# ZihanLiao/pytorch-kaldi-resnet

Hardware: AMD Instinct MI355X
Metric: utterances/sec (300-frame x 80 fbank, bs256/GPU), ResNet-34 + AAM-softmax training step (higher is better)
Workload: dtype f32 (operands as 2 fp16 terms of value x 2^k, 3 cross products, f32 accumulate); 1 GPU; BASELINE configs[1]: ResNet-34 + AAM-softmax (m 0.2, s 30), 1211 speakers, 300-frame x 80 fbank, per-GPU batch 256, fwd+CE+bwd+SGD(0.9, wd 5e-4); global_batch=256, frames=300, feat_dim=80, parallelism=dp1, launch=hipGraph replay (1 graph), mfma=f16x3

## Files before the change

include/spkhip.h:

```cpp
#ifndef SPKHIP_H
#define SPKHIP_H
#include <stddef.h>
#ifdef __cplusplus
extern "C" {
#endif

int spk_version(void);
const char* spk_last_error(void);
int spk_build_flags(void);

#define SPK_IN_AFFINE_RELU 1
#define SPK_EPI_AFFINE 2
#define SPK_EPI_ADD 4
#define SPK_EPI_RELU 8
#define SPK_EPI_STATS 16
#define SPK_IN_BNBWD 64
#define SPK_EPI_BNBWD 32

#define SPK_CONV_WS 128
#define SPK_CONV_PIPE 1024

#define SPK_CONV_M16 (1 << 17)

#define SPK_WGRAD_GROUPS 2048
// ... 77 lines not shown
size_t spk_bn_finalize_workspace(int nblk, int C);
int spk_bn_finalize(const float* partial, int nblk, int C, double count, const float* gamma, const float* beta,
                    float* running_mean, float* running_var, long long* num_batches_tracked, float* mean, float* invstd,
                    float* scale, float* shift, float momentum, float eps, double* ws,
                    const unsigned* amax_in, unsigned* est_out ,
                    void* stream);
int spk_bn_eval_coeffs(const float* gamma, const float* beta, const float* running_mean, const float* running_var,
                       float* scale, float* shift, int C, float eps, void* stream);
int spk_bn_apply(const float* raw, const float* scale, const float* shift, const float* res, const float* res_scale,
                 const float* res_shift, float* out, unsigned* mask_out, long long N, int C, int relu,
                 unsigned* amax_out , void* stream);
int spk_bn_bwd_reduce(const float* dy, const float* raw, const float* act, const float* mean, const float* invstd,
                      const float* scale, const float* shift, float* partial, long long N, int C, int mask_mode,
                      unsigned* chan_amax , void* stream);
int spk_bn_bwd_finalize(const float* partial, int nblk, int C, double count, const float* gamma, const float* invstd,
                        float* dgamma, float* dbeta, float* coef , int accumulate, double* ws,
                        const unsigned* amax_in, const unsigned* raw_amax, const float* mean, unsigned* est_out ,
                        const unsigned* chan_amax ,
                        void* stream);
int spk_bn_bwd_apply(const float* dy, const float* raw, const float* act, const float* mean, const float* invstd,
                     const float* scale, const float* shift, const float* coef, float* draw, float* dz_out, long long N,
                     int C, int mask_mode, unsigned* amax_out ,
                     const unsigned* pair_scale , void* stream);
int spk_absmax(const float* x, unsigned* slot, long long n, void* stream);
int spk_bnbwd_estimate(const float* coef, const float* mean, const float* invstd, int C, const unsigned* amax_in,
                       const unsigned* raw_amax, unsigned* est, void* stream);
int spk_f16_window_count(const float* x, const float* scale, const float* shift, long long n, int C, const unsigned* slot,
                         int pairs, unsigned long long* counts , void* stream);
int spk_affine_estimate(const float* scale, const float* shift, int C, const unsigned* amax_in, unsigned* est, void* stream);

int spk_se_chunks(long long HW);
int spk_se_squeeze(const float* x, float* partial, double* sums , int B, int H, int W, int C, const int* wlen,
                   void* stream);
int spk_se_excite(const double* sums, const float* scale, const float* shift, const float* W1, const float* W2, float* q,
                  float* u, float* g, int B, int C, int Cr, int H, int W, const int* wlen, void* stream);
int spk_se_apply(const float* raw, const float* scale, const float* shift, const float* gate, const float* res,
                 const float* res_scale, const float* res_shift, float* out, unsigned* mask_out, int B, int H, int W, int C,
                 int relu, unsigned* amax_out, const int* wlen, void* stream);
int spk_se_bwd_reduce(const float* dout, const float* raw, const float* act, float* partial, double* S , int B,
                      long long HW, int C, int mask_mode, unsigned* chan_amax, void* stream);
int spk_se_bwd_gate(const double* S, const double* sums, const float* q, const float* u, const float* g, const float* W1,
                    const float* W2, const float* mean, const float* invstd, const float* scale, const float* shift,
                    const float* gamma, float* da, float* du, float* dq, float* dW1, float* dW2, float* dgamma, float* dbeta,
                    float* coef, int accumulate, int B, int C, int Cr, long long HW, const unsigned* amax_in,
                    const unsigned* raw_amax, const unsigned* chan_amax, unsigned* est_out, void* stream);
int spk_se_bwd_apply(const float* dout, const float* raw, const float* act, const float* gate, const float* dqs ,
// ... 118 lines not shown
```

pytorch-kaldi-resnet_amd/csrc/bn.hip:

```cpp
#include "spk_common.h"

enum { MASK_NONE = 0, MASK_ACT = 1, MASK_RAW = 2, MASK_BITS = 3 };

__global__ __launch_bounds__(256) void bn_stats_partial_kernel(const float* __restrict__ x, float* __restrict__ partial,
                                                               long long N, int C, int rows_per_block) {
    __shared__ float red[256][8];
    const int tid = threadIdx.x;
    const int qpr = C >> 2;
    const int quad = tid % qpr, prow = tid / qpr, rstep = 256 / qpr;
    const long long r0 = (long long)blockIdx.x * rows_per_block;
    long long r1 = r0 + rows_per_block;
    if (r1 > N) r1 = N;
    f32x4 s = {0.f, 0.f, 0.f, 0.f}, ss = {0.f, 0.f, 0.f, 0.f};
    for (long long r = r0 + prow; r < r1; r += rstep) {
        const f32x4 v = *(const f32x4*)(x + r * C + quad * 4);
        s += v;
        ss += v * v;
    }
#pragma unroll
    for (int k = 0; k < 4; ++k) {
        red[tid][k] = s[k];
        red[tid][4 + k] = ss[k];
    }
    __syncthreads();
// ... 286 lines not shown
                bits |= __shfl_xor(bits, 4, 64);
                if ((threadIdx.x & 7) == 0) mask_out[i >> 3] = bits;
            }
        }
    }
    if (amax_out) spk_wave_amax_commit(mx, amax_out);
}

extern "C" int spk_bn_apply(const float* raw, const float* scale, const float* shift, const float* res,
                            const float* res_scale, const float* res_shift, float* out, unsigned* mask_out, long long N, int C,
                            int relu, unsigned* amax_out, void* stream) {
    SPK_REQUIRE(raw && scale && shift && out, "spk_bn_apply: null pointer");
    SPK_REQUIRE(N > 0 && bn_c_ok(C), "spk_bn_apply: N=%lld C=%d", N, C);
    SPK_REQUIRE((res_scale == nullptr) == (res_shift == nullptr), "spk_bn_apply: residual affine must come in pairs");
    SPK_REQUIRE(!res_scale || res, "spk_bn_apply: residual affine without residual");
    SPK_REQUIRE(!mask_out || C % 32 == 0, "spk_bn_apply: the sign mask needs C %% 32 == 0 (C=%d)", C);
    const long long nquads = N * C / 4;
    hipLaunchKernelGGL(bn_apply_kernel, dim3(stream_grid(nquads, BN_APPLY_U, BN_APPLY_CAP)), dim3(256), 0, (hipStream_t)stream, raw, scale, shift, res,
                       res_scale, res_shift, out, mask_out, nquads, C, relu, amax_out);
    SPK_LAUNCH_CHECK("spk_bn_apply");
    return 0;
}

__device__ inline f32x4 bn_mask(f32x4 dy, int mode, const float* act, const float* raw_p, f32x4 rawv, f32x4 sc, f32x4 sh,
                                long long off, int C = 0) {
    if (mode == MASK_BITS) {
        const int lg = 31 - __builtin_clz((unsigned)C);
        const long long pix = off >> lg;
        const int c = (int)(off & (C - 1));
        const unsigned bits = ((const unsigned*)act)[pix * (C >> 5) + (c >> 5)] >> (c & 31);
#pragma unroll
        for (int k = 0; k < 4; ++k) dy[k] = ((bits >> k) & 1u) ? dy[k] : 0.f;
    } else if (mode == MASK_ACT) {
        const f32x4 a = *(const f32x4*)(act + off);
#pragma unroll
        for (int k = 0; k < 4; ++k) dy[k] = a[k] > 0.f ? dy[k] : 0.f;
    } else if (mode == MASK_RAW) {
        const f32x4 z = rawv * sc + sh;
#pragma unroll
        for (int k = 0; k < 4; ++k) dy[k] = z[k] > 0.f ? dy[k] : 0.f;
    }
    (void)raw_p;
    return dy;
}

__global__ __launch_bounds__(256) void bn_bwd_reduce_kernel(const float* __restrict__ dy, const float* __restrict__ raw,
                                                            const float* __restrict__ act, const float* __restrict__ mean,
                                                            const float* __restrict__ invstd, const float* __restrict__ scale,
                                                            const float* __restrict__ shift, float* __restrict__ partial,
                                                            long long N, int C, int rows_per_block, int mode,
                                                            unsigned* __restrict__ chan_amax) {
    __shared__ float red[256][8];
    const int tid = threadIdx.x;
    const int qpr = C >> 2;
    const int quad = tid % qpr, prow = tid / qpr, rstep = 256 / qpr;
    const long long r0 = (long long)blockIdx.x * rows_per_block;
    long long r1 = r0 + rows_per_block;
    if (r1 > N) r1 = N;
    const f32x4 mu = *(const f32x4*)(mean + quad * 4), is = *(const f32x4*)(invstd + quad * 4);
    const f32x4 sc = *(const f32x4*)(scale + quad * 4), sh = *(const f32x4*)(shift + quad * 4);
    f32x4 s = {0.f, 0.f, 0.f, 0.f}, ss = {0.f, 0.f, 0.f, 0.f}, mx = {0.f, 0.f, 0.f, 0.f};
    for (long long r = r0 + prow; r < r1; r += rstep) {
        const long long off = r * C + quad * 4;
        const f32x4 rv = ld_stream(raw + off);
        f32x4 d = ld_stream(dy + off);
        d = bn_mask(d, mode, act, raw, rv, sc, sh, off, C);
        const f32x4 xh = (rv - mu) * is;
        s += d;
        ss += d * xh;
#pragma unroll
        for (int k = 0; k < 4; ++k) mx[k] = fmaxf(mx[k], spk_finite_abs(d[k]));
    }
#pragma unroll
    for (int k = 0; k < 4; ++k) {
        red[tid][k] = s[k];
        red[tid][4 + k] = ss[k];
    }
    __syncthreads();
    if (tid < qpr) {
        float a[8];
#pragma unroll
        for (int k = 0; k < 8; ++k) a[k] = 0.f;
        for (int p = 0; p < rstep; ++p)
#pragma unroll
            for (int k = 0; k < 8; ++k) a[k] += red[p * qpr + tid][k];
        float* dst = partial + ((size_t)blockIdx.x * C + tid * 4) * 2;
#pragma unroll
        for (int k = 0; k < 4; ++k) {
            dst[k * 2 + 0] = a[k];
            dst[k * 2 + 1] = a[4 + k];
        }
    }
    if (chan_amax) {
        __syncthreads();
#pragma unroll
        for (int k = 0; k < 4; ++k) red[tid][k] = mx[k];
        __syncthreads();
        if (tid < qpr) {
#pragma unroll
            for (int k = 0; k < 4; ++k) {
                float m = 0.f;
                for (int p = 0; p < rstep; ++p) m = fmaxf(m, red[p * qpr + tid][k]);
                const unsigned bits = __float_as_uint(m);
                unsigned* slot = chan_amax + tid * 4 + k;
                if (bits > __hip_atomic_load(slot, __ATOMIC_RELAXED, __HIP_MEMORY_SCOPE_AGENT)) atomicMax(slot, bits);
            }
        }
    }
}

extern "C" int spk_bn_bwd_reduce(const float* dy, const float* raw, const float* act, const float* mean, const float* invstd,
                                 const float* scale, const float* shift, float* partial, long long N, int C, int mask_mode,
                                 unsigned* chan_amax, void* stream) {
    SPK_REQUIRE(dy && raw && mean && invstd && scale && shift && partial, "spk_bn_bwd_reduce: null pointer");
    SPK_REQUIRE(N > 0 && bn_c_ok(C), "spk_bn_bwd_reduce: N=%lld C=%d", N, C);
    SPK_REQUIRE(mask_mode >= 0 && mask_mode <= 3, "spk_bn_bwd_reduce: mask_mode=%d", mask_mode);
    SPK_REQUIRE((mask_mode != MASK_ACT && mask_mode != MASK_BITS) || act, "spk_bn_bwd_reduce: MASK_ACT / MASK_BITS need the activated tensor / its sign bits");
    const int nb = spk_bn_stats_blocks(N, C);
    const int rpb = (int)((N + nb - 1) / nb);
    hipLaunchKernelGGL(bn_bwd_reduce_kernel, dim3(nb), dim3(256), 0, (hipStream_t)stream, dy, raw, act, mean, invstd, scale,
                       shift, partial, N, C, rpb, mask_mode, chan_amax);
    SPK_LAUNCH_CHECK("spk_bn_bwd_reduce");
    return 0;
}

__device__ inline float bnbwd_bound(float k1, float m1, float m2, float mean, float invstd, float A, float R) {
    const float xh = (R + fabsf(mean)) * fabsf(invstd);
    return fabsf(k1) * (A + fabsf(m1) + xh * fabsf(m2)) * (1.f + 1.52587890625e-05f);
}

template <typename T>
__global__ __launch_bounds__(256) void bn_bwd_finalize_kernel(const T* __restrict__ partial, int nblk, int C, double count,
                                                              const float* __restrict__ gamma, const float* __restrict__ invstd,
                                                              float* __restrict__ dgamma, float* __restrict__ dbeta,
                                                              float* __restrict__ coef, int accumulate,
                                                              const unsigned* __restrict__ amax_in, const unsigned* __restrict__ raw_amax,
                                                              const float* __restrict__ mean, unsigned* __restrict__ est_out,
                                                              const unsigned* __restrict__ chan_amax) {
    __shared__ double red[8][32][2];
    const int tid = threadIdx.x, c = tid & 31, row = tid >> 5;
    const int ch = blockIdx.x * 32 + c;
    double s = 0.0, ss = 0.0;
    if (ch < C) bn_sum_rows<T>(partial, nblk, C, ch, row, s, ss);
    red[row][c][0] = s;
    red[row][c][1] = ss;
// ... 117 lines not shown
            } else
                st_stream(draw + off, o);
            mx = fmaxf(fmaxf(mx, fmaxf(fabsf(o[0]), fabsf(o[1]))), fmaxf(fabsf(o[2]), fabsf(o[3])));
        }
    }
    if (amax_out) spk_wave_amax_commit(mx, amax_out);
}

extern "C" int spk_bn_bwd_apply(const float* dy, const float* raw, const float* act, const float* mean, const float* invstd,
                                const float* scale, const float* shift, const float* coef, float* draw, float* dz_out,
                                long long N, int C, int mask_mode, unsigned* amax_out, const unsigned* pair_scale, void* stream) {
    SPK_REQUIRE(dy && raw && mean && invstd && scale && shift && coef && draw, "spk_bn_bwd_apply: null pointer");
    SPK_REQUIRE(N > 0 && bn_c_ok(C), "spk_bn_bwd_apply: N=%lld C=%d", N, C);
    SPK_REQUIRE(mask_mode >= 0 && mask_mode <= 3, "spk_bn_bwd_apply: mask_mode=%d", mask_mode);
    SPK_REQUIRE((mask_mode != MASK_ACT && mask_mode != MASK_BITS) || act, "spk_bn_bwd_apply: MASK_ACT / MASK_BITS need the activated tensor / its sign bits");
    const long long nquads = N * C / 4;
    SPK_REQUIRE(nquads < 2147483647LL / 8, "spk_bn_bwd_apply: %lld values exceed the 32-bit group index of the kernel", N * C);
    hipLaunchKernelGGL(bn_bwd_apply_kernel, dim3(stream_grid(nquads, BN_BWD_APPLY_U, BN_BWD_APPLY_CAP)), dim3(256), 0, (hipStream_t)stream, dy, raw, act, mean,
                       invstd, scale, shift, coef, draw, dz_out, (unsigned)nquads, C, mask_mode, amax_out, pair_scale);
    SPK_LAUNCH_CHECK("spk_bn_bwd_apply");
    return 0;
}

__global__ __launch_bounds__(256) void absmax_kernel(const float* __restrict__ x, long long n, unsigned* __restrict__ slot) {
    float mx = 0.f;
    const long long nq = n >> 2;
    for (long long i = (long long)blockIdx.x * 256 + threadIdx.x; i < nq; i += (long long)gridDim.x * 256) {
        const f32x4 v = *(const f32x4*)(x + i * 4);
        mx = fmaxf(fmaxf(mx, fmaxf(spk_finite_abs(v[0]), spk_finite_abs(v[1]))), fmaxf(spk_finite_abs(v[2]), spk_finite_abs(v[3])));
    }
    if (blockIdx.x == 0 && threadIdx.x < (n & 3)) mx = fmaxf(mx, spk_finite_abs(x[nq * 4 + threadIdx.x]));
    spk_wave_amax_commit(mx, slot);
}

extern "C" int spk_absmax(const float* x, unsigned* slot, long long n, void* stream) {
    SPK_REQUIRE(x && slot && n > 0, "spk_absmax: bad arguments");
    SPK_REQUIRE((((size_t)x) & 15) == 0, "spk_absmax: x must be 16-byte aligned");
    hipLaunchKernelGGL(absmax_kernel, dim3(stream_grid(n / 4 + 1)), dim3(256), 0, (hipStream_t)stream, x, n, slot);
    SPK_LAUNCH_CHECK("spk_absmax");
    return 0;
}

__global__ __launch_bounds__(256) void bnbwd_estimate_kernel(const float* __restrict__ coef, const float* __restrict__ mean,
                                                             const float* __restrict__ invstd, int C,
                                                             const unsigned* __restrict__ amax_in, const unsigned* __restrict__ raw_amax,
                                                             unsigned* __restrict__ est) {
// ... 117 lines not shown
```

pytorch-kaldi-resnet_amd/engine.py:

```python
import torch

from . import ops
from .hip import MASK_ACT, MASK_BITS, MASK_NONE, MASK_RAW


class _Conv:
    def __init__(self, holder):
        self.h = holder
        self.cin, self.cout, self.k, self.stride = holder.cin, holder.cout, holder.k, holder.stride
        self.wpk = None
        self.wpk_t = None

    def repack(self, need_t):
        w = self.h.weight.data
        if self.cin == 1:
            return
        self.wpk = ops.pack_conv_weight(w, False, self.wpk)
        if need_t:
            self.wpk_t = ops.pack_conv_weight(w, True, self.wpk_t)

    def pack_jobs(self, need_t):
        w = self.h.weight.data
        if self.cin == 1:
            return []
# ... 74 lines not shown
                self.blocks.append(_Block(bp))
        self.head_bn = _BN(model.bn1) if hasattr(model, "bn1") else None
        self.pool_mode = 1 if model.pooling == "mean+std" else 0
        self.dirty = True
        self._packed_for_bwd = False
        self._pack_tables = {}
        self._amax_pool = None
        self._amax_fwd = None
        self._amax_eval = None
        self._fwd_gen = 0
        self.wgrad_stream = None
        self.use_side_stream = True
        self.fuse_bn_reduce = True
        self.fuse_bn_apply = True
        import os
        self.use_sign_masks = os.environ.get("SPK_SIGN_MASKS", "1") == "1"
        self.fuse_apply_min_c = int(os.environ.get("SPK_FUSE_APPLY_MINC", "0"))
        self._fuse_apply_max_c = int(os.environ["SPK_FUSE_APPLY_MAXC"]) if "SPK_FUSE_APPLY_MAXC" in os.environ else None
        self.fuse_apply_1x1 = os.environ.get("SPK_FUSE_APPLY_1X1", "0") == "1"
        self.pair_draw = os.environ.get("SPK_PAIR_DRAW", "1") == "1"
        stem_fused = os.environ.get("SPK_STEM_FUSED", "1")
        self.stem_fused_fwd = stem_fused in ("1", "fwd")
        self.stem_fused_bwd = stem_fused in ("1", "bwd")
        self.chan_amax = os.environ.get("SPK_CHAN_AMAX", "1") == "1"
        self.window_counts = None
        self.bound_log = None

    @property
    def fuse_apply_max_c(self):
        if self._fuse_apply_max_c is not None:
            return self._fuse_apply_max_c
        return 32 if (self.pair_draw and ops.split_for(3, True) == 3) else 1000000

    @fuse_apply_max_c.setter
    def fuse_apply_max_c(self, v):
        self._fuse_apply_max_c = v

    def _all_convs(self):
        for b in self.blocks:
            for c in b.convs:
                yield c
            if b.ds is not None:
                yield b.ds[0]

    def _repack(self, need_t):
        if not self.dirty and (self._packed_for_bwd or not need_t):
# ... 323 lines not shown
                if on_stage_done and (bi == 0 or stage_of[bi - 1] != stage_of[bi]):
                    self._join_wgrad()
                    on_stage_done("layer%d" % stage_of[bi])
            bn = self.stem_bn
            if self.stem_fused_bwd:
                raw0 = saved["raw0"]
                if part is None:
                    part = ops.bn_bwd_partial(d, raw0, None, bn.t4, MASK_RAW)
                coef = ops.bn_bwd_coef(part, raw0.numel() // raw0.shape[-1], bn.h.weight.data, bn.t4, bn.h.weight.grad,
                                       bn.h.bias.grad, accumulate=acc)
                ops.stem_bwd_wgrad(saved["x"], d, raw0, bn.t4, coef, self.stem_conv.h.weight.grad, accumulate=acc)
            else:
                draw0 = ops.bn_backward(d, saved["raw0"], None, bn.t4, bn.h.weight.data, bn.h.weight.grad, bn.h.bias.grad,
                                        MASK_RAW, draw_out=d, accumulate=acc, partial=part)
                ops.stem_wgrad(saved["x"], draw0, self.stem_conv.h.weight.grad, accumulate=acc)
            self._join_wgrad()
            if on_stage_done:
                on_stage_done("stem")

    def _block_bwd(self, b, rec, dout, acc, dout_partial=None, prev=None, dout_amax=None, amx=None, chan=False):
        x, raws, out = rec["x"], rec["raws"], rec["out"]
        n = len(b.convs)
        g, g_part, g_amax, dz = dout, dout_partial, dout_amax, None
        take = (lambda: amx.take()) if amx is not None else (lambda: None)
        for i in range(n - 1, -1, -1):
            c, bn, raw = b.convs[i], b.bns[i], raws[i]
            last = i == n - 1
            inp = x if i == 0 else raws[i - 1]
            in_aff = None if i == 0 else (b.bns[i - 1].t4[2], b.bns[i - 1].t4[3])
            hw = (inp.shape[1], inp.shape[2])
            act = out if last else None
            f16 = amx is not None and ops.split_for(c.k, True) == 3
            add_dz, bnb = False, None
            if i > 0:
                if c.stride == 1 and self.fuse_bn_reduce:
                    bnb = (raws[i - 1], None, b.bns[i - 1].t4)
            elif b.ds is None:
                add_dz = True
                if c.stride == 1 and self.fuse_bn_reduce and prev is not None:
                    bnb = (prev[0], x, prev[1])
                    if rec.get("xmask") is not None:
                        bnb = bnb + (rec["xmask"],)
            res_amax, draw_amax = take(), take()
            pairs = f16 and self.pair_draw
            raw_amax = rec["raw_amax"][i] if f16 else None
            se_last = last and b.se is not None
# ... 28 lines not shown
                    self.bound_log.append((c.cout, c.k, est, draw_amax))
            else:
                lazy_dz = False
                est = take() if pairs else None
                pair = (g_amax, raw_amax, est) if pairs else None
                if se_last:
                    bits = rec.get("mask")
                    lazy_dz = b.ds is None and bits is not None and n > 1
                    ca = amx.take_n(c.cout) if (chan and pairs) else None
                    mode, actm = (MASK_BITS, bits) if bits is not None else (MASK_ACT, out)
                    sums, q, u, gate = rec["se"]
                    S = ops.se_bwd_reduce(g, raw, actm, mode, chan_amax=ca)
                    w1, w2 = b.se.w1, b.se.w2
                    coef, dq, _, _ = ops.se_bwd_gate(S, sums, q, u, gate, w1.data, w2.data, bn.t4, bn.h.weight.data, w1.grad,
                                                     w2.grad, bn.h.weight.grad, bn.h.bias.grad, raw.shape[1] * raw.shape[2],
                                                     accumulate=acc, pair=pair, chan_amax=ca)
                    draw = ops.se_bwd_apply(g, raw, actm, mode, gate, dq[1], bn.t4, coef, e_out=None if lazy_dz else g,
                                            amax_out=draw_amax, pair_scale=est)
                    dz = None if lazy_dz else g
                elif last:
                    bits = rec.get("mask")
                    lazy_dz = b.ds is None and bits is not None and n > 1
                    ca = amx.take_n(c.cout) if (chan and pairs and g_part is None) else None
                    draw = ops.bn_backward(g, raw, bits if bits is not None else out, bn.t4, bn.h.weight.data, bn.h.weight.grad,
                                           bn.h.bias.grad, MASK_BITS if bits is not None else MASK_ACT,
                                           dz_out=None if lazy_dz else g, accumulate=acc, partial=g_part, amax_out=draw_amax,
                                           pair=pair, chan_amax=ca)
                    dz = None if lazy_dz else g
                else:
                    draw = ops.bn_backward(g, raw, None, bn.t4, bn.h.weight.data, bn.h.weight.grad, bn.h.bias.grad, MASK_RAW,
                                           draw_out=g, accumulate=acc, partial=g_part, amax_out=draw_amax, pair=pair)
                draw_slot = est if pairs else draw_amax
                self._count(draw, draw_slot, pairs=pairs)
                if self.bound_log is not None and est is not None:
                    self.bound_log.append((c.cout, c.k, est, draw_amax))
                if add_dz and dz is None and rec.get("mask") is not None:
                    res = ops.conv_dgrad(draw, c.wpk_t, c.cin, c.k, c.stride, hw, add=dout, add_mask=rec["mask"], bn_bwd=bnb,
                                         in_amax=draw_slot if f16 else None, out_amax=res_amax, in_presplit=pairs)
                else:
                    res = ops.conv_dgrad(draw, c.wpk_t, c.cin, c.k, c.stride, hw, add=dz if add_dz else None, bn_bwd=bnb,
                                         in_amax=draw_slot if f16 else None, out_amax=res_amax, in_presplit=pairs)
            g, g_part = res if bnb is not None else (res, None)
            g_amax = res_amax
            self._wgrad(inp, draw, c.h.weight.grad, c.k, c.stride, in_affine=in_aff, accumulate=acc,
                        dy_amax=draw_slot if f16 else None, x_amax=rec["in_amax"][i] if f16 else None, dy_presplit=pairs)
        dx, part, dx_amax = g, g_part, g_amax
        if b.ds is not None:
            cd, bnd = b.ds
            f16d = amx is not None and ops.split_for(1, True) == 3
            drawd_amax = take() if f16d else None
            drawd = ops.bn_backward(dz, rec["rawd"], None, bnd.t4, bnd.h.weight.data, bnd.h.weight.grad, bnd.h.bias.grad,
                                    MASK_NONE, draw_out=dz, accumulate=acc, amax_out=drawd_amax)
            self._count(drawd, drawd_amax)
            self._wgrad(x, drawd, cd.h.weight.grad, 1, cd.stride, accumulate=acc, dy_amax=drawd_amax,
                        x_amax=rec["in_amax"][0] if f16d else None)
            ops.conv_dgrad(drawd, cd.wpk_t, cd.cin, 1, cd.stride, (x.shape[1], x.shape[2]), out=dx, accumulate=True,
                           in_amax=drawd_amax, out_amax=dx_amax)
            part = None
        return dx, part, dx_amax

    def loss_and_grad(self, x, y, on_stage_done=None):
        x = self._check_input(x)
        y = y.contiguous()
        with torch.no_grad():
            logits, saved = self.forward_train(x, y)
            loss_row, dl, rank = ops.softmax_ce(logits, y, grad_scale=1.0 / logits.shape[0])
            loss = ops.mean(loss_row)
        self.backward(saved, dl, on_stage_done)
        return loss, logits, rank


STAGE_ORDER = ["head", "layer4", "layer3", "layer2", "layer1", "stem"]


class GraphedTrainStep:
# ... 116 lines not shown
```

pytorch-kaldi-resnet_amd/hip.py:

```python
import ctypes
import os

import torch

_HERE = os.path.dirname(os.path.abspath(__file__))
LIB_PATH = os.environ.get("SPK_LIB", os.path.join(_HERE, "libspkhip.so"))

IN_AFFINE_RELU, EPI_AFFINE, EPI_ADD, EPI_RELU, EPI_STATS, EPI_BNBWD, IN_BNBWD, CONV_WS = 1, 2, 4, 8, 16, 32, 64, 128
CONV_PIPE = 1024
WGRAD_GROUPS = 2048
IN_PRESPLIT, SIDE_PRESPLIT, DY_PRESPLIT = 1 << 14, 1 << 15, 1 << 16
CONV_M16 = 1 << 17
CONV_CK32 = 1 << 23
WGRAD_NOSHIFT = 1 << 18
WGRAD_M16 = 1 << 19
EPI_WMASK = 1 << 24
PTR_ADD_MASK, PTR_BN_MASK, PTR_IN_MASK, PTR_IN_ACT, PTR_BN_ACT, PTR_SIDE_DZ = 1, 2, 4, 8, 16, 32
MASK_NONE, MASK_ACT, MASK_RAW, MASK_BITS = 0, 1, 2, 3

_P = ctypes.c_void_p
_I = ctypes.c_int
_L = ctypes.c_longlong
_F = ctypes.c_float
_D = ctypes.c_double
# ... 11 lines not shown
    "spk_conv1x1_stream": [_P] * 11 + [_L, _I, _I, _P, _P, _I, _P],
    "spk_conv1x1_stream_rows": [_I, _I],
    "spk_conv_wgrad": [_P] * 6 + [_I] * 16 + [_P, _P, _P],
    "spk_conv_wgrad_limits": [_I, _IP, _IP],
    "spk_wgrad_reduce": [_P, _P, _I, _I, _I, _I, _I, _P],
    "spk_conv_variant_of": [_I, _I, _I, _I, _I],
    "spk_wgrad_variant_of": [_I, _I, _I, _I, _I, _I, _I],
    "spk_stem_fwd_blocks": [_I, _I, _I],
    "spk_stem_conv_fwd": [_P] * 6 + [_I] * 4 + [_P, _P],
    "spk_stem_conv_fwd_len": [_P] * 6 + [_I] * 4 + [_P, _P, _P],
    "spk_stem_wgrad_blocks": [_I, _I, _I],
    "spk_stem_conv_wgrad": [_P] * 4 + [_I] * 4 + [_P],
    "spk_stem_stats": [_P] * 3 + [_I] * 3 + [_P],
    "spk_stem_fwd_apply": [_P] * 8 + [_I] * 3 + [_P],
    "spk_stem_bwd_wgrad": [_P] * 10 + [_I] * 4 + [_P],
    "spk_bn_stats_blocks": [_L, _I],
    "spk_bn_stats_partial": [_P, _P, _L, _I, _P],
    "spk_bn_finalize": [_P, _I, _I, _D] + [_P] * 9 + [_F, _F, _P, _P, _P, _P],
    "spk_bn_eval_coeffs": [_P] * 6 + [_I, _F, _P],
    "spk_bn_apply": [_P] * 8 + [_L, _I, _I, _P, _P],
    "spk_bn_bwd_reduce": [_P] * 8 + [_L, _I, _I, _P, _P],
    "spk_bn_bwd_finalize": [_P, _I, _I, _D] + [_P] * 5 + [_I, _P, _P, _P, _P, _P, _P, _P],
    "spk_bn_bwd_apply": [_P] * 10 + [_L, _I, _I, _P, _P, _P],
    "spk_absmax": [_P, _P, _L, _P],
    "spk_bnbwd_estimate": [_P, _P, _P, _I, _P, _P, _P, _P],
    "spk_f16_window_count": [_P, _P, _P, _L, _I, _P, _I, _P, _P],
    "spk_affine_estimate": [_P, _P, _I, _P, _P, _P],
    "spk_se_chunks": [_L],
    "spk_se_squeeze": [_P, _P, _P, _I, _I, _I, _I, _P, _P],
    "spk_se_excite": [_P] * 8 + [_I] * 5 + [_P, _P],
    "spk_se_apply": [_P] * 9 + [_I] * 5 + [_P, _P, _P],
    "spk_se_bwd_reduce": [_P] * 5 + [_I, _L, _I, _I, _P, _P],
    "spk_se_bwd_gate": [_P] * 20 + [_I] * 4 + [_L] + [_P] * 5,
    "spk_se_bwd_apply": [_P] * 10 + [_I, _L, _I, _I, _P, _P, _P],
    "spk_stats_pool_fwd": [_P, _P, _I, _I, _I, _I, _I, _P],
    "spk_stats_pool_fwd_len": [_P, _P, _P, _I, _I, _I, _I, _I, _P],
    "spk_stats_pool_bwd": [_P, _P, _P, _I, _I, _I, _I, _I, _P, _P],
    "spk_stats_pool_row_form": [_I],
    "spk_stats_pool_row_cap": [],
    "spk_gemm_f32": [_P] * 4 + [_I] * 3 + [_L] * 5 + [_F, _I, _P, _P],
    "spk_gemm_splitk": [_I, _I, _I],
    "spk_colsum": [_P, _P, _I, _I, _I, _P],
    "spk_l2norm_fwd": [_P, _P, _P, _I, _I, _F, _P],
    "spk_l2norm_bwd": [_P, _P, _P, _P, _I, _I, _F, _I, _P],
    "spk_aam_margin_fwd": [_P, _P, _P, _I, _I, _F, _F, _P],
    "spk_aam_margin_bwd": [_P, _P, _P, _P, _I, _I, _F, _F, _P],
# ... 115 lines not shown
```

pytorch-kaldi-resnet_amd/ops.py:

```python
import collections
import ctypes
import os

import torch

from . import hip, tiling
from .hip import (CONV_CK32, CONV_M16, CONV_PIPE, CONV_WS, DY_PRESPLIT, IN_PRESPLIT, SIDE_PRESPLIT, WGRAD_GROUPS, EPI_ADD, EPI_AFFINE, EPI_BNBWD, EPI_RELU,
                  EPI_STATS, EPI_WMASK, IN_AFFINE_RELU, IN_BNBWD, MASK_ACT, MASK_NONE, MASK_RAW,
                  call, ptr, stream)

BN_EPS = 1e-5
BN_MOMENTUM = 0.1

PROFILE = None
_raw_call = call


def call(name, *args, label=None, flops=0.0, nbytes=0.0):
    if PROFILE is None:
        return _raw_call(name, *args)
    e0 = torch.cuda.Event(enable_timing=True)
    e1 = torch.cuda.Event(enable_timing=True)
    e0.record()
    _raw_call(name, *args)
# ... 618 lines not shown
                partial=None, amax_out=None, pair=None, chan_amax=None):
    C = raw.shape[-1]
    N = raw.numel() // C
    coef = torch.empty(3, C, device=raw.device, dtype=torch.float32)
    if partial is None:
        nblk = hip.lib().spk_bn_stats_blocks(N, C)
        part = torch.empty(nblk, C, 2, device=raw.device, dtype=torch.float32)
        call("spk_bn_bwd_reduce", ptr(dy), ptr(raw), ptr(act), ptr(bn4[0]), ptr(bn4[1]), ptr(bn4[2]), ptr(bn4[3]), ptr(part),
             N, C, mask_mode, ptr(chan_amax), stream(), nbytes=_bn_bwd_bytes(raw, mask_mode, 2))
    else:
        assert chan_amax is None, "chan_amax comes out of the reduction pass: partial must be None"
        part, nblk = partial, partial.shape[0]
    call("spk_bn_bwd_finalize", ptr(part), nblk, C, float(N), ptr(gamma), ptr(bn4[1]), ptr(dgamma), ptr(dbeta), ptr(coef),
         1 if accumulate else 0, ptr(_ws64(raw.device)), ptr(pair[0]) if pair else None, ptr(pair[1]) if pair else None,
         ptr(bn4[0]) if pair else None, ptr(pair[2]) if pair else None, ptr(chan_amax) if pair else None, stream())
    if draw_out is None:
        draw_out = torch.empty_like(raw)
    call("spk_bn_bwd_apply", ptr(dy), ptr(raw), ptr(act), ptr(bn4[0]), ptr(bn4[1]), ptr(bn4[2]), ptr(bn4[3]), ptr(coef),
         ptr(draw_out), ptr(dz_out), N, C, mask_mode, ptr(amax_out), ptr(pair[2]) if pair else None, stream(),
         nbytes=_bn_bwd_bytes(raw, mask_mode, 3 + (1 if dz_out is not None else 0)))
    return draw_out


def bn_bwd_coef(partial, count, gamma, bn4, dgamma, dbeta, accumulate=False, amax_in=None, raw_amax=None, est_out=None,
                chan_amax=None):
    C = gamma.numel()
    coef = torch.empty(3, C, device=gamma.device, dtype=torch.float32)
    assert est_out is None or (amax_in is not None and raw_amax is not None)
    call("spk_bn_bwd_finalize", ptr(partial), partial.shape[0], C, float(count), ptr(gamma), ptr(bn4[1]), ptr(dgamma),
         ptr(dbeta), ptr(coef), 1 if accumulate else 0, ptr(_ws64(gamma.device)), ptr(amax_in) if est_out is not None else None,
         ptr(raw_amax) if est_out is not None else None, ptr(bn4[0]) if est_out is not None else None, ptr(est_out),
         ptr(chan_amax) if est_out is not None else None, stream())
    return coef


def bn_bwd_partial(dy, raw, act, bn4, mask_mode, chan_amax=None):
    C = raw.shape[-1]
    N = raw.numel() // C
    nblk = hip.lib().spk_bn_stats_blocks(N, C)
    part = torch.empty(nblk, C, 2, device=raw.device, dtype=torch.float32)
    call("spk_bn_bwd_reduce", ptr(dy), ptr(raw), ptr(act), ptr(bn4[0]), ptr(bn4[1]), ptr(bn4[2]), ptr(bn4[3]), ptr(part),
         N, C, mask_mode, ptr(chan_amax), stream(), nbytes=_bn_bwd_bytes(raw, mask_mode, 2))
    return part


def se_squeeze(x, wlen=None):
# ... 330 lines not shown
```

Before: 5607 utt/s.

## Fuse main and downsample BN backward passes into dual reduce/apply kernels

In residual blocks that have a downsample branch, the backward passes of the last main-path BN and the downsample BN now share one reduction kernel and one apply kernel. Both consume the same masked gradient dz, so dy and the mask are read once instead of being written as dz and reread. The reduce kernel also becomes templated on mask mode with a small row unroll to batch loads. This cuts memory traffic and launches for the few downsample blocks, at the cost of more register pressure and a second BN-backward code path behind SPK_BN_DUAL.

Result: no change. 5641 utt/s (median of 6 runs) (+0.6%).

```diff
diff --git a/include/spkhip.h b/include/spkhip.h
--- a/include/spkhip.h
+++ b/include/spkhip.h
@@ -123,6 +123,13 @@
                      const float* scale, const float* shift, const float* coef, float* draw, float* dz_out, long long N,
                      int C, int mask_mode, unsigned* amax_out ,
                      const unsigned* pair_scale , void* stream);
+int spk_bn_bwd_reduce2(const float* dy, const float* act, const float* raw2, const float* mean2, const float* invstd2,
+                       float* partial2, const float* rawd, const float* meand, const float* invstdd, float* partiald,
+                       long long N, int C, int mask_mode, unsigned* chan_amax, void* stream);
+int spk_bn_bwd_apply2(const float* dy, const float* act, const float* raw2, const float* mean2, const float* invstd2,
+                      const float* coef2, float* draw2, const float* rawd, const float* meand, const float* invstdd,
+                      const float* coefd, float* drawd, long long N, int C, int mask_mode, unsigned* amax2_out,
+                      const unsigned* pair_scale, unsigned* amaxd_out, void* stream);
 int spk_absmax(const float* x, unsigned* slot, long long n, void* stream);
 int spk_bnbwd_estimate(const float* coef, const float* mean, const float* invstd, int C, const unsigned* amax_in,
                        const unsigned* raw_amax, unsigned* est, void* stream);
diff --git a/pytorch-kaldi-resnet_amd/csrc/bn.hip b/pytorch-kaldi-resnet_amd/csrc/bn.hip
--- a/pytorch-kaldi-resnet_amd/csrc/bn.hip
+++ b/pytorch-kaldi-resnet_amd/csrc/bn.hip
@@ -332,76 +332,118 @@
     return 0;
 }
 
-__device__ inline f32x4 bn_mask(f32x4 dy, int mode, const float* act, const float* raw_p, f32x4 rawv, f32x4 sc, f32x4 sh,
-                                long long off, int C = 0) {
-    if (mode == MASK_BITS) {
-        const int lg = 31 - __builtin_clz((unsigned)C);
-        const long long pix = off >> lg;
-        const int c = (int)(off & (C - 1));
-        const unsigned bits = ((const unsigned*)act)[pix * (C >> 5) + (c >> 5)] >> (c & 31);
-#pragma unroll
-        for (int k = 0; k < 4; ++k) dy[k] = ((bits >> k) & 1u) ? dy[k] : 0.f;
-    } else if (mode == MASK_ACT) {
-        const f32x4 a = *(const f32x4*)(act + off);
-#pragma unroll
-        for (int k = 0; k < 4; ++k) dy[k] = a[k] > 0.f ? dy[k] : 0.f;
-    } else if (mode == MASK_RAW) {
-        const f32x4 z = rawv * sc + sh;
-#pragma unroll
-        for (int k = 0; k < 4; ++k) dy[k] = z[k] > 0.f ? dy[k] : 0.f;
-    }
-    (void)raw_p;
-    return dy;
-}
-
+#ifndef BN_BWD_REDUCE_U
+#define BN_BWD_REDUCE_U 4
+#endif
+static __device__ __forceinline__ void bn_bwd_fold(float (*red)[8], f32x4 s, f32x4 ss, float* __restrict__ partial, int C,
+                                                   int qpr, int rstep) {
+    const int tid = threadIdx.x;
+#pragma unroll
+    for (int k = 0; k < 4; ++k) {
+        red[tid][k] = s[k];
+        red[tid][4 + k] = ss[k];
+    }
+    __syncthreads();
+    if (tid < qpr) {
+        float a[8];
+#pragma unroll
+        for (int k = 0; k < 8; ++k) a[k] = 0.f;
+        for (int p = 0; p < rstep; ++p)
+#pragma unroll
+            for (int k = 0; k < 8; ++k) a[k] += red[p * qpr + tid][k];
+        float* dst = partial + ((size_t)blockIdx.x * C + tid * 4) * 2;
+#pragma unroll
+        for (int k = 0; k < 4; ++k) {
+            dst[k * 2 + 0] = a[k];
+            dst[k * 2 + 1] = a[4 + k];
+        }
+    }
+}
+
+template <int MODE, bool DUAL, bool MAIN>
 __global__ __launch_bounds__(256) void bn_bwd_reduce_kernel(const float* __restrict__ dy, const float* __restrict__ raw,
                                                             const float* __restrict__ act, const float* __restrict__ mean,
                                                             const float* __restrict__ invstd, const float* __restrict__ scale,
                                                             const float* __restrict__ shift, float* __restrict__ partial,
-                                                            long long N, int C, int rows_per_block, int mode,
+                                                            const float* __restrict__ rawd, const float* __restrict__ meand,
+                                                            const float* __restrict__ invstdd, float* __restrict__ partiald,
+                                                            long long N, int C, int rows_per_block,
                                                             unsigned* __restrict__ chan_amax) {
+    static_assert(MAIN || DUAL, "nothing to reduce");
+    static_assert(!DUAL || MODE == MASK_BITS || MODE == MASK_ACT, "the shared dz is the masked gradient of a block output");
     __shared__ float red[256][8];
+    constexpr int U = BN_BWD_REDUCE_U;
     const int tid = threadIdx.x;
     const int qpr = C >> 2;
     const int quad = tid % qpr, prow = tid / qpr, rstep = 256 / qpr;
     const long long r0 = (long long)blockIdx.x * rows_per_block;
     long long r1 = r0 + rows_per_block;
     if (r1 > N) r1 = N;
-    const f32x4 mu = *(const f32x4*)(mean + quad * 4), is = *(const f32x4*)(invstd + quad * 4);
-    const f32x4 sc = *(const f32x4*)(scale + quad * 4), sh = *(const f32x4*)(shift + quad * 4);
-    f32x4 s = {0.f, 0.f, 0.f, 0.f}, ss = {0.f, 0.f, 0.f, 0.f}, mx = {0.f, 0.f, 0.f, 0.f};
-    for (long long r = r0 + prow; r < r1; r += rstep) {
-        const long long off = r * C + quad * 4;
-        const f32x4 rv = ld_stream(raw + off);
-        f32x4 d = ld_stream(dy + off);
-        d = bn_mask(d, mode, act, raw, rv, sc, sh, off, C);
-        const f32x4 xh = (rv - mu) * is;
-        s += d;
-        ss += d * xh;
-#pragma unroll
-        for (int k = 0; k < 4; ++k) mx[k] = fmaxf(mx[k], spk_finite_abs(d[k]));
-    }
-#pragma unroll
-    for (int k = 0; k < 4; ++k) {
-        red[tid][k] = s[k];
-        red[tid][4 + k] = ss[k];
-    }
-    __syncthreads();
-    if (tid < qpr) {
-        float a[8];
-#pragma unroll
-        for (int k = 0; k < 8; ++k) a[k] = 0.f;
-        for (int p = 0; p < rstep; ++p)
-#pragma unroll
-            for (int k = 0; k < 8; ++k) a[k] += red[p * qpr + tid][k];
-        float* dst = partial + ((size_t)blockIdx.x * C + tid * 4) * 2;
-#pragma unroll
-        for (int k = 0; k < 4; ++k) {
-            dst[k * 2 + 0] = a[k];
-            dst[k * 2 + 1] = a[4 + k];
-        }
-    }
-    if (chan_amax) {
+    const f32x4 zero = {0.f, 0.f, 0.f, 0.f};
+    f32x4 mu = zero, is = zero, sc = zero, sh = zero, mud = zero, isd = zero;
+    if (MAIN) {
+        mu = *(const f32x4*)(mean + quad * 4);
+        is = *(const f32x4*)(invstd + quad * 4);
+    }
+    if (MODE == MASK_RAW) {
+        sc = *(const f32x4*)(scale + quad * 4);
+        sh = *(const f32x4*)(shift + quad * 4);
+    }
+    if (DUAL) {
+        mud = *(const f32x4*)(meand + quad * 4);
+        isd = *(const f32x4*)(invstdd + quad * 4);
+    }
+    const int cw = C >> 5, wq = (quad * 4) >> 5, wsh = (quad * 4) & 31;
+    f32x4 s = zero, ss = zero, ssd = zero, mx = zero;
+    for (long long r = r0 + prow; r < r1; r += (long long)rstep * U) {
+        f32x4 rv[U], dv[U], rd[U], av[U];
+        unsigned mw[U];
+#pragma unroll
+        for (int u = 0; u < U; ++u) {
+            const long long ru = r + (long long)rstep * u;
+            const long long rr = ru < r1 ? ru : r;
+            const long long off = rr * C + quad * 4;
+            if (MAIN) rv[u] = ld_stream(raw + off);
+            dv[u] = ld_stream(dy + off);
+            if (DUAL) rd[u] = ld_stream(rawd + off);
+            if (MODE == MASK_BITS) mw[u] = ((const unsigned*)act)[rr * cw + wq];
+            else if (MODE == MASK_ACT) av[u] = *(const f32x4*)(act + off);
+        }
+#pragma unroll
+        for (int u = 0; u < U; ++u) {
+            if (r + (long long)rstep * u >= r1) continue;
+            f32x4 d = dv[u];
+            if (MODE == MASK_BITS) {
+                const unsigned bits = mw[u] >> wsh;
+#pragma unroll
+                for (int k = 0; k < 4; ++k) d[k] = ((bits >> k) & 1u) ? d[k] : 0.f;
+            } else if (MODE == MASK_ACT) {
+#pragma unroll
+                for (int k = 0; k < 4; ++k) d[k] = av[u][k] > 0.f ? d[k] : 0.f;
+            } else if (MODE == MASK_RAW) {
+                const f32x4 z = rv[u] * sc + sh;
+#pragma unroll
+                for (int k = 0; k < 4; ++k) d[k] = z[k] > 0.f ? d[k] : 0.f;
+            }
+            s += d;
+            if (MAIN) {
+                const f32x4 xh = (rv[u] - mu) * is;
+                ss += d * xh;
+#pragma unroll
+                for (int k = 0; k < 4; ++k) mx[k] = fmaxf(mx[k], spk_finite_abs(d[k]));
+            }
+            if (DUAL) {
+                const f32x4 xhd = (rd[u] - mud) * isd;
+                ssd += d * xhd;
+            }
+        }
+    }
+    if (MAIN) bn_bwd_fold(red, s, ss, partial, C, qpr, rstep);
+    if (DUAL) {
+        if (MAIN) __syncthreads();
+        bn_bwd_fold(red, s, ssd, partiald, C, qpr, rstep);
+    }
+    if (MAIN && chan_amax) {
         __syncthreads();
 #pragma unroll
         for (int k = 0; k < 4; ++k) red[tid][k] = mx[k];
@@ -417,6 +459,23 @@
             }
         }
     }
+}
+
+template <bool DUAL, bool MAIN>
+static void bn_bwd_reduce_launch(int mode, int nb, hipStream_t st, const float* dy, const float* raw, const float* act,
+                                 const float* mean, const float* invstd, const float* scale, const float* shift, float* partial,
+                                 const float* rawd, const float* meand, const float* invstdd, float* partiald, long long N, int C,
+                                 int rpb, unsigned* chan_amax) {
+#define BN_BWD_REDUCE_CASE(M)                                                                                                    \
+    hipLaunchKernelGGL((bn_bwd_reduce_kernel<M, DUAL, MAIN>), dim3(nb), dim3(256), 0, st, dy, raw, act, mean, invstd, scale,      \
+                       shift, partial, rawd, meand, invstdd, partiald, N, C, rpb, chan_amax)
+    if (mode == MASK_BITS) BN_BWD_REDUCE_CASE(MASK_BITS);
+    else if (mode == MASK_ACT) BN_BWD_REDUCE_CASE(MASK_ACT);
+    else if constexpr (!DUAL) {
+        if (mode == MASK_RAW) BN_BWD_REDUCE_CASE(MASK_RAW);
+        else BN_BWD_REDUCE_CASE(MASK_NONE);
+    }
+#undef BN_BWD_REDUCE_CASE
 }
 
 extern "C" int spk_bn_bwd_reduce(const float* dy, const float* raw, const float* act, const float* mean, const float* invstd,
@@ -428,9 +487,30 @@
     SPK_REQUIRE((mask_mode != MASK_ACT && mask_mode != MASK_BITS) || act, "spk_bn_bwd_reduce: MASK_ACT / MASK_BITS need the activated tensor / its sign bits");
     const int nb = spk_bn_stats_blocks(N, C);
     const int rpb = (int)((N + nb - 1) / nb);
-    hipLaunchKernelGGL(bn_bwd_reduce_kernel, dim3(nb), dim3(256), 0, (hipStream_t)stream, dy, raw, act, mean, invstd, scale,
-                       shift, partial, N, C, rpb, mask_mode, chan_amax);
+    bn_bwd_reduce_launch<false, true>(mask_mode, nb, (hipStream_t)stream, dy, raw, act, mean, invstd, scale, shift, partial,
+                                      nullptr, nullptr, nullptr, nullptr, N, C, rpb, chan_amax);
     SPK_LAUNCH_CHECK("spk_bn_bwd_reduce");
+    return 0;
+}
+
+extern "C" int spk_bn_bwd_reduce2(const float* dy, const float* act, const float* raw2, const float* mean2, const float* invstd2,
+                                  float* partial2, const float* rawd, const float* meand, const float* invstdd, float* partiald,
+                                  long long N, int C, int mask_mode, unsigned* chan_amax, void* stream) {
+    SPK_REQUIRE(dy && act && rawd && meand && invstdd && partiald, "spk_bn_bwd_reduce2: null pointer");
+    SPK_REQUIRE(!partial2 || (raw2 && mean2 && invstd2), "spk_bn_bwd_reduce2: partial2 needs raw2, mean2 and invstd2");
+    SPK_REQUIRE(!chan_amax || partial2, "spk_bn_bwd_reduce2: chan_amax comes with the main path's sums (partial2)");
+    SPK_REQUIRE(N > 0 && bn_c_ok(C), "spk_bn_bwd_reduce2: N=%lld C=%d", N, C);
+    SPK_REQUIRE(mask_mode == MASK_ACT || (mask_mode == MASK_BITS && C % 32 == 0),
+                "spk_bn_bwd_reduce2: mask_mode=%d C=%d (MASK_ACT, or MASK_BITS with C %% 32 == 0)", mask_mode, C);
+    const int nb = spk_bn_stats_blocks(N, C);
+    const int rpb = (int)((N + nb - 1) / nb);
+    if (partial2)
+        bn_bwd_reduce_launch<true, true>(mask_mode, nb, (hipStream_t)stream, dy, raw2, act, mean2, invstd2, nullptr, nullptr,
+                                         partial2, rawd, meand, invstdd, partiald, N, C, rpb, chan_amax);
+    else
+        bn_bwd_reduce_launch<true, false>(mask_mode, nb, (hipStream_t)stream, dy, nullptr, act, nullptr, nullptr, nullptr, nullptr,
+                                          nullptr, rawd, meand, invstdd, partiald, N, C, rpb, nullptr);
+    SPK_LAUNCH_CHECK("spk_bn_bwd_reduce2");
     return 0;
 }
 
@@ -594,6 +674,80 @@
     return 0;
 }
 
+#ifndef BN_BWD_APPLY2_CAP
+#define BN_BWD_APPLY2_CAP 1536
+#endif
+__global__ __launch_bounds__(256) void bn_bwd_apply2_kernel(const float* dy, const float* __restrict__ act,
+                                                            const float* __restrict__ raw2, const float* __restrict__ mean2,
+                                                            const float* __restrict__ invstd2, const float* __restrict__ coef2,
+                                                            float* __restrict__ draw2, const float* __restrict__ rawd,
+                                                            const float* __restrict__ meand, const float* __restrict__ invstdd,
+                                                            const float* __restrict__ coefd, float* drawd, unsigned nquads, int C,
+                                                            int mode, unsigned* __restrict__ amax2_out,
+                                                            const unsigned* __restrict__ pair_scale,
+                                                            unsigned* __restrict__ amaxd_out) {
+    const int cmask = C - 1;
+    float mx2 = 0.f, mxd = 0.f;
+    const float sig = pair_scale ? spk_sigma_from_amax_bits(*pair_scale) : 1.f;
+    const unsigned stride = gridDim.x * 256u;
+    const int lgq = 29 - __builtin_clz((unsigned)C);
+    const unsigned cw = (unsigned)C >> 5;
+    const int c0 = (threadIdx.x * 4) & cmask;
+    const f32x4 pmu2 = *(const f32x4*)(mean2 + c0), pis2 = *(const f32x4*)(invstd2 + c0), pk12 = *(const f32x4*)(coef2 + c0);
+    const f32x4 pm12 = *(const f32x4*)(coef2 + C + c0), pm22 = *(const f32x4*)(coef2 + 2 * C + c0);
+    const f32x4 pmud = *(const f32x4*)(meand + c0), pisd = *(const f32x4*)(invstdd + c0), pk1d = *(const f32x4*)(coefd + c0);
+    const f32x4 pm1d = *(const f32x4*)(coefd + C + c0), pm2d = *(const f32x4*)(coefd + 2 * C + c0);
+    for (unsigned i = blockIdx.x * 256u + threadIdx.x; i < nquads; i += stride) {
+        const size_t off = (size_t)i * 4;
+        const f32x4 rv2 = ld_stream(raw2 + off);
+        const f32x4 rvd = ld_stream(rawd + off);
+        f32x4 d = ld_stream(dy + off);
+        if (mode == MASK_BITS) {
+            const unsigned bits = ((const unsigned*)act)[(size_t)(i >> lgq) * cw + ((unsigned)c0 >> 5)] >> (c0 & 31);
+#pragma unroll
+            for (int k = 0; k < 4; ++k) d[k] = ((bits >> k) & 1u) ? d[k] : 0.f;
+        } else {
+            const f32x4 av = *(const f32x4*)(act + off);
+#pragma unroll
+            for (int k = 0; k < 4; ++k) d[k] = av[k] > 0.f ? d[k] : 0.f;
+        }
+        const f32x4 xh2 = (rv2 - pmu2) * pis2;
+        const f32x4 o2 = pk12 * (d - pm12 - xh2 * pm22);
+        const f32x4 xhd = (rvd - pmud) * pisd;
+        const f32x4 od = pk1d * (d - pm1d - xhd * pm2d);
+        if (pair_scale) {
+            uint2 t0, t1;
+            split2h(o2, sig, t0, t1);
+            st_stream(draw2 + off, spk_pair_pack(t0, t1));
+        } else
+            st_stream(draw2 + off, o2);
+        st_stream(drawd + off, od);
+        mx2 = fmaxf(fmaxf(mx2, fmaxf(fabsf(o2[0]), fabsf(o2[1]))), fmaxf(fabsf(o2[2]), fabsf(o2[3])));
+        mxd = fmaxf(fmaxf(mxd, fmaxf(fabsf(od[0]), fabsf(od[1]))), fmaxf(fabsf(od[2]), fabsf(od[3])));
+    }
+    if (amax2_out) spk_wave_amax_commit(mx2, amax2_out);
+    if (amaxd_out) spk_wave_amax_commit(mxd, amaxd_out);
+}
+
+extern "C" int spk_bn_bwd_apply2(const float* dy, const float* act, const float* raw2, const float* mean2, const float* invstd2,
+                                 const float* coef2, float* draw2, const float* rawd, const float* meand, const float* invstdd,
+                                 const float* coefd, float* drawd, long long N, int C, int mask_mode, unsigned* amax2_out,
+                                 const unsigned* pair_scale, unsigned* amaxd_out, void* stream) {
+    SPK_REQUIRE(dy && act && raw2 && mean2 && invstd2 && coef2 && draw2 && rawd && meand && invstdd && coefd && drawd,
+                "spk_bn_bwd_apply2: null pointer");
+    SPK_REQUIRE(N > 0 && bn_c_ok(C), "spk_bn_bwd_apply2: N=%lld C=%d", N, C);
+    SPK_REQUIRE(mask_mode == MASK_ACT || (mask_mode == MASK_BITS && C % 32 == 0),
+                "spk_bn_bwd_apply2: mask_mode=%d C=%d (MASK_ACT, or MASK_BITS with C %% 32 == 0)", mask_mode, C);
+    SPK_REQUIRE(draw2 != dy && draw2 != drawd, "spk_bn_bwd_apply2: draw2 must be a buffer of its own (drawd may be dy)");
+    const long long nquads = N * C / 4;
+    SPK_REQUIRE(nquads < 2147483647LL / 8, "spk_bn_bwd_apply2: %lld values exceed the 32-bit group index of the kernel", N * C);
+    hipLaunchKernelGGL(bn_bwd_apply2_kernel, dim3(stream_grid(nquads, 1, BN_BWD_APPLY2_CAP)), dim3(256), 0, (hipStream_t)stream, dy,
+                       act, raw2, mean2, invstd2, coef2, draw2, rawd, meand, invstdd, coefd, drawd, (unsigned)nquads, C, mask_mode,
+                       amax2_out, pair_scale, amaxd_out);
+    SPK_LAUNCH_CHECK("spk_bn_bwd_apply2");
+    return 0;
+}
+
 __global__ __launch_bounds__(256) void absmax_kernel(const float* __restrict__ x, long long n, unsigned* __restrict__ slot) {
     float mx = 0.f;
     const long long nq = n >> 2;
diff --git a/pytorch-kaldi-resnet_amd/engine.py b/pytorch-kaldi-resnet_amd/engine.py
--- a/pytorch-kaldi-resnet_amd/engine.py
+++ b/pytorch-kaldi-resnet_amd/engine.py
@@ -120,6 +120,7 @@
         stem_fused = os.environ.get("SPK_STEM_FUSED", "1")
         self.stem_fused_fwd = stem_fused in ("1", "fwd")
         self.stem_fused_bwd = stem_fused in ("1", "bwd")
+        self.bn_dual = os.environ.get("SPK_BN_DUAL", "1") == "1"
         self.chan_amax = os.environ.get("SPK_CHAN_AMAX", "1") == "1"
         self.window_counts = None
         self.bound_log = None
@@ -489,6 +490,7 @@
         x, raws, out = rec["x"], rec["raws"], rec["out"]
         n = len(b.convs)
         g, g_part, g_amax, dz = dout, dout_partial, dout_amax, None
+        drawd, drawd_amax = None, None
         take = (lambda: amx.take()) if amx is not None else (lambda: None)
         for i in range(n - 1, -1, -1):
             c, bn, raw = b.convs[i], b.bns[i], raws[i]
@@ -563,11 +565,21 @@
                     bits = rec.get("mask")
                     lazy_dz = b.ds is None and bits is not None and n > 1
                     ca = amx.take_n(c.cout) if (chan and pairs and g_part is None) else None
-                    draw = ops.bn_backward(g, raw, bits if bits is not None else out, bn.t4, bn.h.weight.data, bn.h.weight.grad,
-                                           bn.h.bias.grad, MASK_BITS if bits is not None else MASK_ACT,
-                                           dz_out=None if lazy_dz else g, accumulate=acc, partial=g_part, amax_out=draw_amax,
-                                           pair=pair, chan_amax=ca)
-                    dz = None if lazy_dz else g
+                    if b.ds is not None and self.bn_dual:
+                        bnd = b.ds[1]
+                        drawd_amax = take() if (amx is not None and ops.split_for(1, True) == 3) else None
+                        draw, drawd = ops.bn_backward2(g, bits if bits is not None else out,
+                                                       MASK_BITS if bits is not None else MASK_ACT, raw, bn.t4, bn.h.weight.data,
+                                                       bn.h.weight.grad, bn.h.bias.grad, rec["rawd"], bnd.t4, bnd.h.weight.data,
+                                                       bnd.h.weight.grad, bnd.h.bias.grad, drawd_out=g, accumulate=acc,
+                                                       partial=g_part, amax_out=draw_amax, pair=pair, chan_amax=ca,
+                                                       amaxd_out=drawd_amax)
+                    else:
+                        draw = ops.bn_backward(g, raw, bits if bits is not None else out, bn.t4, bn.h.weight.data,
+                                               bn.h.weight.grad, bn.h.bias.grad, MASK_BITS if bits is not None else MASK_ACT,
+                                               dz_out=None if lazy_dz else g, accumulate=acc, partial=g_part, amax_out=draw_amax,
+                                               pair=pair, chan_amax=ca)
+                        dz = None if lazy_dz else g
                 else:
                     draw = ops.bn_backward(g, raw, None, bn.t4, bn.h.weight.data, bn.h.weight.grad, bn.h.bias.grad, MASK_RAW,
                                            draw_out=g, accumulate=acc, partial=g_part, amax_out=draw_amax, pair=pair)
@@ -589,9 +601,10 @@
         if b.ds is not None:
             cd, bnd = b.ds
             f16d = amx is not None and ops.split_for(1, True) == 3
-            drawd_amax = take() if f16d else None
-            drawd = ops.bn_backward(dz, rec["rawd"], None, bnd.t4, bnd.h.weight.data, bnd.h.weight.grad, bnd.h.bias.grad,
-                                    MASK_NONE, draw_out=dz, accumulate=acc, amax_out=drawd_amax)
+            if drawd is None:
+                drawd_amax = take() if f16d else None
+                drawd = ops.bn_backward(dz, rec["rawd"], None, bnd.t4, bnd.h.weight.data, bnd.h.weight.grad, bnd.h.bias.grad,
+                                        MASK_NONE, draw_out=dz, accumulate=acc, amax_out=drawd_amax)
             self._count(drawd, drawd_amax)
             self._wgrad(x, drawd, cd.h.weight.grad, 1, cd.stride, accumulate=acc, dy_amax=drawd_amax,
                         x_amax=rec["in_amax"][0] if f16d else None)
diff --git a/pytorch-kaldi-resnet_amd/hip.py b/pytorch-kaldi-resnet_amd/hip.py
--- a/pytorch-kaldi-resnet_amd/hip.py
+++ b/pytorch-kaldi-resnet_amd/hip.py
@@ -57,6 +57,8 @@
     "spk_bn_bwd_reduce": [_P] * 8 + [_L, _I, _I, _P, _P],
     "spk_bn_bwd_finalize": [_P, _I, _I, _D] + [_P] * 5 + [_I, _P, _P, _P, _P, _P, _P, _P],
     "spk_bn_bwd_apply": [_P] * 10 + [_L, _I, _I, _P, _P, _P],
+    "spk_bn_bwd_reduce2": [_P] * 10 + [_L, _I, _I, _P, _P],
+    "spk_bn_bwd_apply2": [_P] * 12 + [_L, _I, _I, _P, _P, _P, _P],
     "spk_absmax": [_P, _P, _L, _P],
     "spk_bnbwd_estimate": [_P, _P, _P, _I, _P, _P, _P, _P],
     "spk_f16_window_count": [_P, _P, _P, _L, _I, _P, _I, _P, _P],
diff --git a/pytorch-kaldi-resnet_amd/ops.py b/pytorch-kaldi-resnet_amd/ops.py
--- a/pytorch-kaldi-resnet_amd/ops.py
+++ b/pytorch-kaldi-resnet_amd/ops.py
@@ -664,6 +664,50 @@
     return draw_out
 
 
+def bn_bwd_partial2(dy, act, mask_mode, raw2, bn4_2, rawd, bn4_d, want_main=True, chan_amax=None):
+    C = raw2.shape[-1]
+    N = raw2.numel() // C
+    assert rawd.shape == raw2.shape and (want_main or chan_amax is None)
+    nblk = hip.lib().spk_bn_stats_blocks(N, C)
+    part2 = torch.empty(nblk, C, 2, device=raw2.device, dtype=torch.float32) if want_main else None
+    partd = torch.empty(nblk, C, 2, device=raw2.device, dtype=torch.float32)
+    call("spk_bn_bwd_reduce2", ptr(dy), ptr(act), ptr(raw2) if want_main else None, ptr(bn4_2[0]) if want_main else None,
+         ptr(bn4_2[1]) if want_main else None, ptr(part2), ptr(rawd), ptr(bn4_d[0]), ptr(bn4_d[1]), ptr(partd), N, C, mask_mode,
+         ptr(chan_amax), stream(), nbytes=_bn_bwd_bytes(raw2, mask_mode, 3 if want_main else 2))
+    return part2, partd
+
+
+def bn_bwd_apply2(dy, act, mask_mode, raw2, bn4_2, coef2, rawd, bn4_d, coefd, drawd_out=None, amax_out=None, pair_scale=None,
+                  amaxd_out=None):
+    C = raw2.shape[-1]
+    N = raw2.numel() // C
+    draw2 = torch.empty_like(raw2)
+    if drawd_out is None:
+        drawd_out = torch.empty_like(rawd)
+    call("spk_bn_bwd_apply2", ptr(dy), ptr(act), ptr(raw2), ptr(bn4_2[0]), ptr(bn4_2[1]), ptr(coef2), ptr(draw2), ptr(rawd),
+         ptr(bn4_d[0]), ptr(bn4_d[1]), ptr(coefd), ptr(drawd_out), N, C, mask_mode, ptr(amax_out), ptr(pair_scale),
+         ptr(amaxd_out), stream(), nbytes=_bn_bwd_bytes(raw2, mask_mode, 5))
+    return draw2, drawd_out
+
+
+def bn_backward2(dy, act, mask_mode, raw2, bn4_2, gamma2, dgamma2, dbeta2, rawd, bn4_d, gammad, dgammad, dbetad, drawd_out=None,
+                 accumulate=False, partial=None, amax_out=None, pair=None, chan_amax=None, amaxd_out=None):
+    C = raw2.shape[-1]
+    N = raw2.numel() // C
+    assert partial is None or chan_amax is None, "chan_amax comes out of the reduction pass: partial must be None"
+    part2, partd = bn_bwd_partial2(dy, act, mask_mode, raw2, bn4_2, rawd, bn4_d, want_main=partial is None, chan_amax=chan_amax)
+    if partial is not None:
+        part2 = partial
+    coef2 = torch.empty(3, C, device=raw2.device, dtype=torch.float32)
+    call("spk_bn_bwd_finalize", ptr(part2), part2.shape[0], C, float(N), ptr(gamma2), ptr(bn4_2[1]), ptr(dgamma2), ptr(dbeta2),
+         ptr(coef2), 1 if accumulate else 0, ptr(_ws64(raw2.device)), ptr(pair[0]) if pair else None,
+         ptr(pair[1]) if pair else None, ptr(bn4_2[0]) if pair else None, ptr(pair[2]) if pair else None,
+         ptr(chan_amax) if pair else None, stream())
+    coefd = bn_bwd_coef(partd, N, gammad, bn4_d, dgammad, dbetad, accumulate)
+    return bn_bwd_apply2(dy, act, mask_mode, raw2, bn4_2, coef2, rawd, bn4_d, coefd, drawd_out=drawd_out, amax_out=amax_out,
+                         pair_scale=pair[2] if pair else None, amaxd_out=amaxd_out)
+
+
 def bn_bwd_coef(partial, count, gamma, bn4, dgamma, dbeta, accumulate=False, amax_in=None, raw_amax=None, est_out=None,
                 chan_amax=None):
     C = gamma.numel()
```
